# tsnorri/vcf2multialign

Hardware: AMD Instinct MI355X
Metric: aligned A2M Gbases/sec (higher is better)
Workload: dtype u8

## Files before the change

### vcf2multialign_amd/csrc/kernels.hpp

```cpp
#pragma once

#include <hip/hip_runtime.h>
#include <stdint.h>

#ifdef V2M_CHECKED_BUILD
__device__ uint32_t v2m_lds_poison_seed;
#endif

namespace v2m {

typedef uint32_t u32;
typedef uint64_t u64;

constexpr int kWave = 64;
typedef u32 vec4u __attribute__((ext_vector_type(4)));
typedef vec4u vec4u_unaligned8 __attribute__((aligned(8)));

#ifdef V2M_CHECKED_BUILD
__device__ __forceinline__ u32 poison_hash(u32 seed, u32 wg, u32 i)
{
	u32 h = seed ^ (wg * 0x9E3779B1u) ^ (i * 0x85EBCA77u);
	h ^= h >> 15; h *= 0x2C1B3C6Du;
	h ^= h >> 12; h *= 0x297A2D39u;
	h ^= h >> 15;
// ... 1065 lines not shown
		if (lane == 0) excl = 0;
		u32 const chunk_max = __shfl(incl, 63, kWave);

		u32 run = excl > cur ? excl : cur;
		bool uncertain = false;
		for (u64 m = w; m; m &= m - 1) {
			u32 const e = wi * 64u + __builtin_ctzll(m);
			edge_span const sp = spans[e];
			uncertain |= sp.src < run;
			run = sp.tgt > run ? sp.tgt : run;
		}

		u64 out = w;
		if (__any(uncertain)) {
			out = 0;
			u32 c = cur;
			u64 busy = __ballot(w != 0);
			while (busy) {
				int const j = __builtin_ctzll(busy);
				busy &= busy - 1;
				if (lane == j) {
					for (u64 m = w; m; m &= m - 1) {
						int const b = __builtin_ctzll(m);
						edge_span const sp = spans[wi * 64u + b];
						if (sp.src >= c) {
							out |= 1ULL << b;
							c = sp.tgt;
						}
					}
				}
				c = __shfl(c, j, kWave);
			}
			cur = c;
		} else {
			cur = chunk_max > cur ? chunk_max : cur;
		}
		if (wi < word_end)
			eff_row[wi] = out;
	}
}


struct tile_tables {
	u32 const *edge_begin;
	u32 const *cross_offsets;
	u32 const *cross_edges;
};

template <typename LabelPtr>
__device__ __forceinline__ void fill_patch_bytes(
	unsigned char *tile, u32 tile_base, u32 aln_begin, u32 label_len, LabelPtr label,
	u32 from, u32 to, u32 start, u32 step, char gap)
{
	for (u32 pos = from + start; pos < to; pos += step) {
		u32 const off = pos - aln_begin;
		tile[pos - tile_base] = (off < label_len) ? (unsigned char) label[off] : (unsigned char) gap;
	}
}

constexpr int kCandLds = 512;
constexpr int kLabelLds = 1024;
constexpr int kGroupRowsLds = 16;
constexpr int kEffWordsLds = kCandLds / 64 + 2;
constexpr int kLongQueueLds = 16;

struct cached_patch {
	unsigned short begin_rel;
	unsigned short span;
	unsigned short label_rel;
	unsigned short label_len;
};

struct patch_cache {
	cached_patch patch[kCandLds];
	u64 eff[kGroupRowsLds][kEffWordsLds];
	unsigned char labels[kLabelLds];
	u32 long_queue[kLongQueueLds];
	u32 long_count;
};

struct tile_job {
	u32 tile_base, tile_end;
	u32 cross_begin, n_cross, range_begin, n_range;
	u32 n_lds;
	u32 w0;
};

__device__ __forceinline__ void load_eff_cache(
	patch_cache &pc, tile_job const &job, u64 const *__restrict__ eff, u64 eff_words_per_row, u32 first_row, u32 n_rows, int t)
{
	if (0 == job.n_lds) return;
	u32 const nw = ((job.range_begin + job.n_lds - 1) >> 6) - job.w0 + 1;
	u32 const rows = n_rows < (u32) kGroupRowsLds ? n_rows : (u32) kGroupRowsLds;
	for (u32 i = t; i < rows * nw; i += kSpliceThreads)
		pc.eff[i / nw][i % nw] = eff[(u64) (first_row + i / nw) * eff_words_per_row + job.w0 + i % nw];
}

template <bool kWindow = false, bool kSet = false>
__device__ __forceinline__ void load_patch_cache(
	patch_cache &pc, tile_job &job, tile_tables const &tt, edge_patch const *__restrict__ patches, char const *__restrict__ labels,
	u64 const *__restrict__ eff, u64 eff_words_per_row, u32 tile, u32 row_begin, u32 n_group_rows, int t, u32 col_base = 0, u32 col_end = 0,
	set_tile_tables const st = set_tile_tables{})
{
	if (kSet) {
		job.tile_base = st.col_begin[tile];
		job.tile_end = st.col_end[tile];
	} else {
		job.tile_base = (kWindow ? col_base : 0u) + tile * (u32) kTileBytes;
		job.tile_end = (kWindow && col_end - job.tile_base < (u32) kTileBytes) ? col_end : job.tile_base + kTileBytes;
	}
	job.cross_begin = tt.cross_offsets[tile];
	job.n_cross = tt.cross_offsets[tile + 1] - job.cross_begin;
	job.range_begin = tt.edge_begin[tile];
	job.n_range = (kSet ? st.edge_end[tile] : tt.edge_begin[tile + 1]) - job.range_begin;
	job.n_lds = job.n_range < (u32) kCandLds ? job.n_range : (u32) kCandLds;
	job.w0 = job.range_begin >> 6;
	if (job.n_lds) {
		u32 const label_base = patches[job.range_begin].label_begin;
		for (u32 i = t; i < job.n_lds; i += kSpliceThreads) {
			edge_patch const p = patches[job.range_begin + i];
			u32 const span = p.aln_end - p.aln_begin, rel = p.label_begin - label_base;
			cached_patch c;
			c.begin_rel = (unsigned short) (p.aln_begin - job.tile_base);
			c.span = span < 0xFFFFu ? (unsigned short) span : (unsigned short) 0xFFFF;
			bool const label_ok = rel + p.label_len <= (u32) kLabelLds;
			c.label_rel = label_ok ? (unsigned short) rel : (unsigned short) 0xFFFF;
			c.label_len = label_ok ? (unsigned short) p.label_len : (unsigned short) 0;
			pc.patch[i] = c;
		}
		edge_patch const last = patches[job.range_begin + job.n_lds - 1];
		u32 const label_span = last.label_begin + last.label_len - label_base;
		u32 const label_len = label_span < (u32) kLabelLds ? label_span : (u32) kLabelLds;
		for (u32 i = t; i < label_len; i += kSpliceThreads)
			pc.labels[i] = (unsigned char) labels[label_base + i];
	}
	load_eff_cache(pc, job, eff, eff_words_per_row, row_begin, n_group_rows, t);
	if (t == 0) pc.long_count = 0;
}

struct tile_patch {
	u32 edge;
	u32 aln_begin;
	u32 from, to;
	u32 label_len;
	u32 label_begin;
	bool in_lds;
};

__device__ __forceinline__ u32 candidate_edge(tile_job const &job, tile_tables const &tt, u32 i)
{
	return (i < job.n_cross) ? tt.cross_edges[job.cross_begin + i] : job.range_begin + (i - job.n_cross);
}

__device__ __forceinline__ bool candidate_in_lds(tile_job const &job, u32 i)
{
	return i >= job.n_cross && i - job.n_cross < job.n_lds;
}

template <bool kWindow = false>
__device__ __forceinline__ tile_patch candidate_patch(
	patch_cache const &pc, tile_job const &job, edge_patch const *__restrict__ patches, u32 i, u32 e, bool cached)
{
	u32 const tile_end = kWindow ? job.tile_end : job.tile_base + kTileBytes;
	cached_patch c{};
	if (cached) {
		c = pc.patch[i - job.n_cross];
		cached = c.span != 0xFFFF && c.label_rel != 0xFFFF;
	}
	tile_patch tp;
	tp.edge = e;
	if (cached) {
		tp.aln_begin = tp.from = job.tile_base + c.begin_rel;
		tp.to = tp.from + c.span < tile_end ? tp.from + c.span : tile_end;
		tp.label_len = c.label_len;
		tp.label_begin = c.label_rel;
		tp.in_lds = true;
	} else {
		edge_patch const p = patches[e];
		tp.aln_begin = p.aln_begin;
		tp.from = p.aln_begin > job.tile_base ? p.aln_begin : job.tile_base;
		tp.to = p.aln_end < tile_end ? p.aln_end : tile_end;
		tp.label_len = p.label_len;
		tp.label_begin = p.label_begin;
		tp.in_lds = false;
	}
	return tp;
}

__device__ __forceinline__ bool candidate_effective(
	patch_cache const &pc, tile_job const &job, tile_tables const &tt, u64 const *__restrict__ eff_row, u32 local_row, u32 i,
	u32 &e, bool &cached)
{
	cached = candidate_in_lds(job, i) && local_row < (u32) kGroupRowsLds;
	if (cached) {
		e = job.range_begin + (i - job.n_cross);
		return (pc.eff[local_row][(e >> 6) - job.w0] >> (e & 63)) & 1;
	}
	e = candidate_edge(job, tt, i);
	return (eff_row[e >> 6] >> (e & 63)) & 1;
}

template <bool kWindow, typename F>
__device__ __forceinline__ void for_each_effective_candidate(
	patch_cache const &pc, tile_job const &job, tile_tables const &tt, edge_patch const *__restrict__ patches,
	u64 const *__restrict__ eff_row, u32 local_row, int t, F &&f)
{
	u32 const n_cand = job.n_cross + job.n_range;
	for (u32 i = t; i < n_cand; i += kSpliceThreads) {
		u32 e;
		bool cached;
		if (!candidate_effective(pc, job, tt, eff_row, local_row, i, e, cached)) continue;
		f(candidate_patch<kWindow>(pc, job, patches, i, e, cached));
	}
}

template <bool kWindow = false>
__device__ __forceinline__ void patch_row_tile(
	unsigned char *buf, patch_cache &pc, tile_job const &job, tile_tables const &tt,
	edge_patch const *__restrict__ patches, char const *__restrict__ labels,
	u64 const *__restrict__ eff_row, u32 local_row, int t, char gap)
{
	u32 const tile_end = kWindow ? job.tile_end : job.tile_base + kTileBytes;
	for_each_effective_candidate<kWindow>(pc, job, tt, patches, eff_row, local_row, t, [&](tile_patch const &tp) {
		if (tp.to - tp.from > kLongPatch) {
			u32 const slot = atomicAdd(&pc.long_count, 1u);
			if (slot < (u32) kLongQueueLds) { pc.long_queue[slot] = tp.edge; return; }
		}
		if (tp.in_lds)
			fill_patch_bytes(buf, job.tile_base, tp.aln_begin, tp.label_len, pc.labels + tp.label_begin, tp.from, tp.to, 0, 1, gap);
		else
			fill_patch_bytes(buf, job.tile_base, tp.aln_begin, tp.label_len, labels + tp.label_begin, tp.from, tp.to, 0, 1, gap);
	});
	__syncthreads();

	u32 const n_long = pc.long_count < (u32) kLongQueueLds ? pc.long_count : (u32) kLongQueueLds;
	if (n_long) {
		for (u32 q = t >> 6; q < n_long; q += kSpliceThreads >> 6) {
			edge_patch const p = patches[pc.long_queue[q]];
			u32 const from = p.aln_begin > job.tile_base ? p.aln_begin : job.tile_base;
			u32 const to = p.aln_end < tile_end ? p.aln_end : tile_end;
			fill_patch_bytes(buf, job.tile_base, p.aln_begin, p.label_len, labels + p.label_begin, from, to, t & 63, 64, gap);
		}
		__syncthreads();
		if (t == 0) pc.long_count = 0;
	}
	V2M_POISON_LDS_RANGE(pc.long_queue, 0u, (u32) kLongQueueLds);
}

__device__ __forceinline__ void map_block(u32 b, u32 n_groups, u32 n_tiles, u32 tile_run, u32 &tile, u32 &group)
{
	u32 const per_super = tile_run * n_groups;
	u32 const super = b / per_super, within = b % per_super;
	u32 const t0 = super * tile_run;
	u32 const run = (n_tiles - t0 < tile_run) ? n_tiles - t0 : tile_run;
	group = within / run;
	tile = t0 + within % run;
}

__device__ __forceinline__ u32 set_tile_chunks(set_tile_tables const &st, u32 tile)
{
	return (st.col_end[tile] - st.col_begin[tile] + 15u) >> 4;
}

template <bool kNonTemporal, bool kWindow, bool kSet = false>
__device__ __forceinline__ void splice_aligned_tiles(
	vec4u const *__restrict__ tmpl, u64 const *__restrict__ eff, u64 eff_words_per_row,
	tile_tables tt, edge_patch const *__restrict__ patches, char const *__restrict__ labels,
	char *__restrict__ out, u64 row_pitch, u32 n_rows, u32 rows_per_group, u32 n_groups, u32 n_tiles, u32 tile_run,
	u64 store_limit, char gap, u32 col_base, u32 col_end, set_tile_tables const st = set_tile_tables{})
{
	__shared__ vec4u lds[2][kTileChunks];
	__shared__ patch_cache pc;

	int const t = threadIdx.x;
	u32 tile, group;
	map_block(blockIdx.x, n_groups, n_tiles, tile_run, tile, group);
	u32 const row_begin = group * rows_per_group;
	u32 const row_end = (row_begin + rows_per_group < n_rows) ? row_begin + rows_per_group : n_rows;
	V2M_POISON_LDS(lds);
	V2M_POISON_LDS(pc);

	u32 const n_chunks = kSet ? set_tile_chunks(st, tile) : (u32) kTileChunks;
	u32 const record_offset = kSet ? st.record_offset[tile] : 0u;
	vec4u pristine[kChunksPerThread];
#pragma unroll
	for (int k = 0; k < kChunksPerThread; ++k) {
		if (kSet) pristine[k] = (u32) (t + kSpliceThreads * k) < n_chunks ? tmpl[(record_offset >> 4) + t + kSpliceThreads * k] : vec4u{0, 0, 0, 0};
		else pristine[k] = tmpl[(u64) tile * kTileChunks + t + kSpliceThreads * k];
	}

	tile_job job;
	load_patch_cache<kWindow, kSet>(pc, job, tt, patches, labels, eff, eff_words_per_row, tile, row_begin, row_end - row_begin, t, col_base, col_end, st);
	u32 const tile_base = job.tile_base;

	for (u32 row = row_begin; row < row_end; ++row) {
		vec4u *const buf = lds[(row - row_begin) & 1];
		u32 const cached_row = (row - row_begin) % (u32) kGroupRowsLds;
		if (row != row_begin && 0 == cached_row)
			load_eff_cache(pc, job, eff, eff_words_per_row, row, row_end - row, t);
#pragma unroll
		for (int k = 0; k < kChunksPerThread; ++k)
			if (!kSet || (u32) (t + kSpliceThreads * k) < n_chunks) buf[t + kSpliceThreads * k] = pristine[k];
		__syncthreads();

		patch_row_tile<kWindow>((unsigned char *) buf, pc, job, tt, patches, labels, eff + (u64) row * eff_words_per_row, cached_row, t, gap);

		char *const dst = out + (u64) row * row_pitch + (kSet ? (u64) record_offset : (u64) tile * kTileBytes);
#pragma unroll
		for (int k = 0; k < kChunksPerThread; ++k) {
			int const c = t + kSpliceThreads * k;
			if (kSet ? (u32) c < n_chunks : (kWindow ? (u64) tile * kTileBytes : (u64) tile_base) + (u64) c * 16 < store_limit) {
				vec4u const nv = buf[c];
				if (kNonTemporal)
					__builtin_nontemporal_store(nv, (vec4u *) (dst + c * 16));
				else
					*(vec4u *) (dst + c * 16) = nv;
			}
		}
	}
}

template <bool kNonTemporal>
__global__ __launch_bounds__(kSpliceThreads) void splice_aligned_kernel(
	vec4u const *__restrict__ tmpl, u64 const *__restrict__ eff, u64 eff_words_per_row,
	tile_tables tt, edge_patch const *__restrict__ patches, char const *__restrict__ labels,
	char *__restrict__ out, u64 row_pitch, u32 n_rows, u32 rows_per_group, u32 n_groups, u32 n_tiles, u32 tile_run,
	u64 store_limit , char gap)
{
	splice_aligned_tiles<kNonTemporal, false>(tmpl, eff, eff_words_per_row, tt, patches, labels, out, row_pitch, n_rows, rows_per_group, n_groups,
		n_tiles, tile_run, store_limit, gap, 0u, 0u);
}

template <bool kNonTemporal>
__global__ __launch_bounds__(kSpliceThreads) void splice_aligned_window_kernel(
	vec4u const *__restrict__ tmpl, u64 const *__restrict__ eff, u64 eff_words_per_row,
	tile_tables tt, edge_patch const *__restrict__ patches, char const *__restrict__ labels,
	char *__restrict__ out, u64 row_pitch, u32 n_rows, u32 rows_per_group, u32 n_groups, u32 n_tiles, u32 tile_run,
	u64 store_limit, char gap, u32 col_base, u32 col_end)
{
	splice_aligned_tiles<kNonTemporal, true>(tmpl, eff, eff_words_per_row, tt, patches, labels, out, row_pitch, n_rows, rows_per_group, n_groups,
		n_tiles, tile_run, store_limit, gap, col_base, col_end);
}

template <bool kNonTemporal>
__global__ __launch_bounds__(kSpliceThreads) void splice_aligned_set_kernel(
	vec4u const *__restrict__ tmpl, u64 const *__restrict__ eff, u64 eff_words_per_row,
	tile_tables tt, set_tile_tables st, edge_patch const *__restrict__ patches, char const *__restrict__ labels,
	char *__restrict__ out, u64 row_pitch, u32 n_rows, u32 rows_per_group, u32 n_groups, u32 n_tiles, u32 tile_run, char gap)
{
	splice_aligned_tiles<kNonTemporal, true, true>(tmpl, eff, eff_words_per_row, tt, patches, labels, out, row_pitch, n_rows, rows_per_group, n_groups,
		n_tiles, tile_run, 0, gap, 0u, 0u, st);
}


__device__ __forceinline__ u32 zero_bytes_mask(u32 x)
{
	return ~(((x & 0x7F7F7F7Fu) + 0x7F7F7F7Fu) | x | 0x7F7F7F7Fu);
}

__device__ __forceinline__ u32 wave_inclusive_scan_u32(u32 v)
{
	v += (u32) __builtin_amdgcn_update_dpp(0, (int) v, 0x111, 0xf, 0xf, false);
	v += (u32) __builtin_amdgcn_update_dpp(0, (int) v, 0x112, 0xf, 0xf, false);
	v += (u32) __builtin_amdgcn_update_dpp(0, (int) v, 0x114, 0xf, 0xf, false);
	v += (u32) __builtin_amdgcn_update_dpp(0, (int) v, 0x118, 0xf, 0xf, false);
	v += (u32) __builtin_amdgcn_update_dpp(0, (int) v, 0x142, 0xa, 0xf, false);
	v += (u32) __builtin_amdgcn_update_dpp(0, (int) v, 0x143, 0xc, 0xf, false);
	return v;
}

// ... 38 lines not shown
	u32 *__restrict__ tile_counts , u32 n_tiles,
	u32 n_rows, u32 rows_per_group, u32 n_groups, u32 tile_run, u32 col_base, u32 col_end, set_tile_tables const st = set_tile_tables{})
{
	__shared__ vec4u lds[kTileChunks];
	__shared__ patch_cache pc;
	__shared__ int row_delta[kCountRowsMax];
	__shared__ int cand_delta[kCandDeltaLds];
	__shared__ u32 wave_sums[kSpliceThreads / 64];

	int const t = threadIdx.x;
	u32 tile, group;
	map_block(blockIdx.x, n_groups, n_tiles, tile_run, tile, group);
	u32 const row_begin = group * rows_per_group;
	u32 const row_end = (row_begin + rows_per_group < n_rows) ? row_begin + rows_per_group : n_rows;
	V2M_POISON_LDS(lds);
	V2M_POISON_LDS(pc);
	V2M_POISON_LDS(row_delta);
	V2M_POISON_LDS(cand_delta);
	V2M_POISON_LDS(wave_sums);

	u32 const n_chunks = kSet ? set_tile_chunks(st, tile) : (u32) kTileChunks;
	u32 mine = 0;
#pragma unroll
	for (int k = 0; k < kChunksPerThread; ++k) {
		if (kSet && (u32) (t + kSpliceThreads * k) >= n_chunks) continue;
		vec4u const v = tmpl0[(kSet ? (u64) (st.record_offset[tile] >> 4) : (u64) tile * kTileChunks) + t + kSpliceThreads * k];
		lds[t + kSpliceThreads * k] = v;
#pragma unroll
		for (int d = 0; d < 4; ++d)
			mine += 4 - __builtin_popcount(zero_bytes_mask(v[d]));
	}
#pragma unroll
	for (int d = 32; d >= 1; d >>= 1) mine += __shfl_down(mine, d, kWave);
	if ((t & 63) == 0) wave_sums[t >> 6] = mine;
	for (u32 r = t; r < (u32) kCountRowsMax; r += kSpliceThreads) row_delta[r] = 0;

	tile_job job;
	load_patch_cache<kWindow, kSet>(pc, job, tt, patches, labels, eff, eff_words_per_row, tile, row_begin, row_end - row_begin, t, col_base, col_end, st);
	__syncthreads();
	u32 tile_count = 0;
#pragma unroll
	for (int wv = 0; wv < kSpliceThreads / 64; ++wv) tile_count += wave_sums[wv];

	unsigned char const *const tile_bytes = (unsigned char const *) lds;
	auto patch_delta = [&](tile_patch const &tp) {
		u32 const label_end = tp.aln_begin + tp.label_len;
		int const label_in_tile = label_end > tp.from ? (int) ((label_end < tp.to ? label_end : tp.to) - tp.from) : 0;
		return label_in_tile - (int) count_nonzero_bytes(tile_bytes, tp.from - job.tile_base, tp.to - job.tile_base);
	};
	u32 const n_cand = job.n_cross + job.n_range;
	for (u32 i = t; i < n_cand && i < (u32) kCandDeltaLds; i += kSpliceThreads)
		cand_delta[i] = patch_delta(candidate_patch<kWindow>(pc, job, patches, i, candidate_edge(job, tt, i), candidate_in_lds(job, i)));
	__syncthreads();
	for (u32 sub = row_begin; sub < row_end; sub += kGroupRowsLds) {
		u32 const sub_end = sub + kGroupRowsLds < row_end ? sub + kGroupRowsLds : row_end;
		if (sub != row_begin) {
			asm volatile("s_waitcnt lgkmcnt(0)" ::: "memory");
			__syncthreads();
			load_eff_cache(pc, job, eff, eff_words_per_row, sub, sub_end - sub, t);
			__syncthreads();
		}
		u32 const sub_rows = sub_end - sub;
		u32 const nw = job.n_lds ? ((job.range_begin + job.n_lds - 1) >> 6) - job.w0 + 1 : 0;
		for (u32 idx = t; idx < sub_rows * nw; idx += kSpliceThreads) {
			u32 const r = idx / nw, w = idx % nw;
			u32 const first = (job.w0 + w) * 64u;
			u64 bits = pc.eff[r][w];
			if (first < job.range_begin) bits &= ~0ULL << (job.range_begin - first);
			u32 const cached_end = job.range_begin + job.n_lds;
			if (cached_end < first + 64u) bits &= (1ULL << (cached_end - first)) - 1;
			int delta = 0;
			for (; bits; bits &= bits - 1) {
				u32 const e = first + (u32) __builtin_ctzll(bits);
				u32 const i = job.n_cross + (e - job.range_begin);
				delta += i < (u32) kCandDeltaLds ? cand_delta[i] : patch_delta(candidate_patch<kWindow>(pc, job, patches, i, e, true));
			}
			if (delta) atomicAdd(&row_delta[sub - row_begin + r], delta);
		}
		u32 const n_other = n_cand - job.n_lds;
		for (u32 idx = t; idx < sub_rows * n_other; idx += kSpliceThreads) {
			u32 const r = idx / n_other, j = idx % n_other;
			u32 const i = j < job.n_cross ? j : j + job.n_lds;
			u32 const e = candidate_edge(job, tt, i);
			if (!((eff[(u64) (sub + r) * eff_words_per_row + (e >> 6)] >> (e & 63)) & 1)) continue;
			int const delta = i < (u32) kCandDeltaLds ? cand_delta[i] : patch_delta(candidate_patch<kWindow>(pc, job, patches, i, e, false));
			if (delta) atomicAdd(&row_delta[sub - row_begin + r], delta);
		}
	}
	__syncthreads();
	for (u32 r = t; r < row_end - row_begin; r += kSpliceThreads)
		tile_counts[(u64) (row_begin + r) * n_tiles + tile] = (u32) ((int) tile_count + row_delta[r]);
}

__global__ __launch_bounds__(kSpliceThreads) void count_unaligned_kernel(
	vec4u const *__restrict__ tmpl0, u64 const *__restrict__ eff, u64 eff_words_per_row,
	tile_tables tt, edge_patch const *__restrict__ patches, char const *__restrict__ labels,
	u32 *__restrict__ tile_counts , u32 n_tiles,
	u32 n_rows, u32 rows_per_group, u32 n_groups, u32 tile_run)
{
	count_unaligned_tiles<false>(tmpl0, eff, eff_words_per_row, tt, patches, labels, tile_counts, n_tiles, n_rows, rows_per_group, n_groups, tile_run, 0u, 0u);
}

__global__ __launch_bounds__(kSpliceThreads) void count_unaligned_window_kernel(
	vec4u const *__restrict__ tmpl0, u64 const *__restrict__ eff, u64 eff_words_per_row,
	tile_tables tt, edge_patch const *__restrict__ patches, char const *__restrict__ labels,
	u32 *__restrict__ tile_counts , u32 n_tiles,
	u32 n_rows, u32 rows_per_group, u32 n_groups, u32 tile_run, u32 col_base, u32 col_end)
{
	count_unaligned_tiles<true>(tmpl0, eff, eff_words_per_row, tt, patches, labels, tile_counts, n_tiles, n_rows, rows_per_group, n_groups, tile_run, col_base, col_end);
}

__global__ __launch_bounds__(kSpliceThreads) void count_unaligned_set_kernel(
// ... 174 lines not shown
	if (c & 4) { *(u32_unaligned *) p = (u32) rest; p += 4; rest >>= 32; }
	if (c & 2) { *(u16_unaligned *) p = (u16) rest; p += 2; rest >>= 16; }
	if (c & 1) *p = (char) rest;
}

template <bool kNonTemporal, u32 kQueue, bool kWindow, bool kSet = false>
__device__ __forceinline__ void splice_unaligned_tiles(
	vec4u const *__restrict__ tmpl0, u64 const *__restrict__ eff, u64 eff_words_per_row,
	tile_tables tt, edge_patch const *__restrict__ patches, char const *__restrict__ labels,
	u32 const *__restrict__ tile_offsets , u32 n_tiles,
	char *__restrict__ out, u64 row_pitch, u32 n_rows, u32 rows_per_group, u32 n_groups, u32 tile_run, u32 col_base, u32 col_end,
	set_tile_tables const st = set_tile_tables{})
{
	constexpr int kWaves = kSpliceThreads / 64, kSlots = kChunksPerThread * kWaves;
	__shared__ vec4u lds[kTileChunks];
	__shared__ patch_cache pc;
	__shared__ __attribute__((aligned(16))) u32 wave_sums[kSlots];
	__shared__ u32 compact_sel[16];
	__shared__ vec4u queue_data[kQueue];
	__shared__ u32 queue_desc[kQueue];
	__shared__ u32 queue_count;

	V2M_POISON_LDS(lds);
	V2M_POISON_LDS(pc);
	V2M_POISON_LDS(wave_sums);
	V2M_POISON_LDS(compact_sel);
	V2M_POISON_LDS(queue_data);
	V2M_POISON_LDS(queue_desc);
	V2M_POISON_LDS(queue_count);
	int const t = threadIdx.x;
	int const lane = t & 63, wave = __builtin_amdgcn_readfirstlane(t >> 6);
	if (t < 16) compact_sel[t] = compaction_selector((u32) t);
	u32 tile, group;
	map_block(blockIdx.x, n_groups, n_tiles, tile_run, tile, group);
	{
		u32 const t0 = tile / tile_run * tile_run;
		u32 const run = (n_tiles - t0 < tile_run) ? n_tiles - t0 : tile_run;
		if (0 == run % 8) { u32 const j = tile - t0; tile = t0 + (j & 7) * (run / 8) + (j >> 3); }
	}
	u32 const row_begin = group * rows_per_group;
	u32 const row_end = (row_begin + rows_per_group < n_rows) ? row_begin + rows_per_group : n_rows;

	u32 const n_chunks = kSet ? set_tile_chunks(st, tile) : (u32) kTileChunks;
	vec4u pristine[kChunksPerThread];
#pragma unroll
	for (int k = 0; k < kChunksPerThread; ++k) {
		if (kSet) pristine[k] = (u32) (t + kSpliceThreads * k) < n_chunks ? tmpl0[(st.record_offset[tile] >> 4) + t + kSpliceThreads * k] : vec4u{0, 0, 0, 0};
		else pristine[k] = tmpl0[(u64) tile * kTileChunks + t + kSpliceThreads * k];
	}

	tile_job job;
	load_patch_cache<kWindow, kSet>(pc, job, tt, patches, labels, eff, eff_words_per_row, tile, row_begin, row_end - row_begin, t, col_base, col_end, st);

	char *dst_prev = out;
	for (u32 row = row_begin; ; ++row) {
		bool const past_end = row >= row_end;
		u32 const tile_offset = past_end ? 0u : tile_offsets[(u64) row * n_tiles + tile];
		if (!past_end) {
			if (row != row_begin && 0 == (row - row_begin) % (u32) kGroupRowsLds)
				load_eff_cache(pc, job, eff, eff_words_per_row, row, row_end - row, t);
#pragma unroll
			for (int k = 0; k < kChunksPerThread; ++k)
				if (!kSet || (u32) (t + kSpliceThreads * k) < n_chunks) lds[t + kSpliceThreads * k] = pristine[k];
		}
		asm volatile("s_waitcnt lgkmcnt(0)" ::: "memory");
		__syncthreads();

		if (row != row_begin) {
			u32 const n = (u32) __builtin_amdgcn_readfirstlane((int) queue_count);
			V2M_POISON_LDS_RANGE(queue_desc, n < kQueue ? n : kQueue, kQueue);
			V2M_POISON_LDS_RANGE(queue_data, n < kQueue ? n : kQueue, kQueue);
			for (u32 pass = 0; 64 * pass < n; ++pass) {
				if (((row + pass) & (u32) (kWaves - 1)) != (u32) wave) continue;
				u32 const idx = 64 * pass + (u32) lane;
				if (idx < n) {
					u32 const e = queue_desc[idx];
					pack_chunk_and_store_exact(queue_data[idx], e & 15u, dst_prev + (e >> 4), compact_sel);
				}
			}
		}
		if (past_end) break;

		patch_row_tile<kWindow>((unsigned char *) lds, pc, job, tt, patches, labels, eff + (u64) row * eff_words_per_row, (row - row_begin) % (u32) kGroupRowsLds, t, 0);

		vec4u v[kChunksPerThread];
		u32 mine[kChunksPerThread], incl[kChunksPerThread];
#pragma unroll
		for (int k = 0; k < kChunksPerThread; ++k) {
			if (kSet) v[k] = (u32) (t + kSpliceThreads * k) < n_chunks ? lds[t + kSpliceThreads * k] : vec4u{0, 0, 0, 0};
			else v[k] = lds[t + kSpliceThreads * k];
		}
#pragma unroll
		for (int k = 0; k < kChunksPerThread; ++k) {
			u32 bytes = 0;
#pragma unroll
			for (int d = 0; d < 4; ++d) bytes = __builtin_amdgcn_msad_u8(v[k][d] ^ 0x01010101u, v[k][d], bytes);
			incl[k] = mine[k] = bytes | (bytes - 1u < 15u ? 0x10000u : 0u);
		}
		wave_inclusive_scan_u32_lockstep(incl);
		if (lane == 63) {
			vec4u sums;
#pragma unroll
			for (int k = 0; k < kChunksPerThread; ++k) sums[k] = incl[k];
			*(vec4u *) &wave_sums[kChunksPerThread * wave] = sums;
		}
		__syncthreads();

		u32 slot_end = lane < kSlots ? wave_sums[kChunksPerThread * (lane % kWaves) + lane / kWaves] : 0u;
		slot_end += (u32) __builtin_amdgcn_update_dpp(0, (int) slot_end, 0x111, 0xf, 0xf, false);
		slot_end += (u32) __builtin_amdgcn_update_dpp(0, (int) slot_end, 0x112, 0xf, 0xf, false);
		slot_end += (u32) __builtin_amdgcn_update_dpp(0, (int) slot_end, 0x114, 0xf, 0xf, false);
		slot_end += (u32) __builtin_amdgcn_update_dpp(0, (int) slot_end, 0x118, 0xf, 0xf, false);

		char *const dst = out + (u64) row * row_pitch + tile_offset;
		u32 const n_fit = (u32) __builtin_popcountll(__ballot(lane < kSlots && (slot_end >> 16) <= kQueue));
		u32 const n_queued = n_fit ? (u32) __builtin_amdgcn_readlane((int) slot_end, (int) n_fit - 1) >> 16 : 0u;
		u32 offs[kChunksPerThread];
		u32 dense = 0;
#pragma unroll
		for (int k = 0; k < kChunksPerThread; ++k) {
			int const slot = k * kWaves + wave;
			u32 const slot_begin = slot ? (u32) __builtin_amdgcn_readlane((int) slot_end, slot - 1) : 0u;
			u32 const c = mine[k] & 0xFFFFu;
			u32 const before = slot_begin + incl[k] - mine[k];
			u32 const off = before & 0xFFFFu;
			offs[k] = off;
			if (16 == c) {
				if (kNonTemporal) __builtin_nontemporal_store(v[k], (vec4u_unaligned *) (dst + off));
				else *(vec4u_unaligned *) (dst + off) = v[k];
			}
			if ((u32) slot < n_fit) {
				if (mine[k] >> 16) {
					u32 const pos = before >> 16;
					queue_desc[pos] = c | off << 4;
					queue_data[pos] = v[k];
				}
			}
			else dense |= 1u << k;
		}
		for (; dense; dense &= dense - 1) {
			u32 const j = (u32) __builtin_ctz(dense);
			u32 const c = (0 == j ? mine[0] : 1 == j ? mine[1] : 2 == j ? mine[2] : mine[3]) & 0xFFFFu;
			u32 const o = 0 == j ? offs[0] : 1 == j ? offs[1] : 2 == j ? offs[2] : offs[3];
			if (c - 1u < 15u) pack_chunk_and_store_exact(lds[(u32) t + (u32) kSpliceThreads * j], c, dst + o, compact_sel);
		}
		if (0 == t) queue_count = n_queued;
		dst_prev = dst;
	}
}

template <bool kNonTemporal, u32 kQueue = 128>
__global__ __launch_bounds__(kSpliceThreads) void splice_unaligned_kernel(
	vec4u const *__restrict__ tmpl0, u64 const *__restrict__ eff, u64 eff_words_per_row,
	tile_tables tt, edge_patch const *__restrict__ patches, char const *__restrict__ labels,
	u32 const *__restrict__ tile_offsets , u32 n_tiles,
	char *__restrict__ out, u64 row_pitch, u32 n_rows, u32 rows_per_group, u32 n_groups, u32 tile_run)
{
	splice_unaligned_tiles<kNonTemporal, kQueue, false>(tmpl0, eff, eff_words_per_row, tt, patches, labels, tile_offsets, n_tiles, out, row_pitch,
		n_rows, rows_per_group, n_groups, tile_run, 0u, 0u);
}

template <bool kNonTemporal>
__global__ __launch_bounds__(kSpliceThreads) void splice_unaligned_window_kernel(
	vec4u const *__restrict__ tmpl0, u64 const *__restrict__ eff, u64 eff_words_per_row,
	tile_tables tt, edge_patch const *__restrict__ patches, char const *__restrict__ labels,
	u32 const *__restrict__ tile_offsets, u32 n_tiles,
	char *__restrict__ out, u64 row_pitch, u32 n_rows, u32 rows_per_group, u32 n_groups, u32 tile_run, u32 col_base, u32 col_end)
{
	splice_unaligned_tiles<kNonTemporal, 128, true>(tmpl0, eff, eff_words_per_row, tt, patches, labels, tile_offsets, n_tiles, out, row_pitch,
		n_rows, rows_per_group, n_groups, tile_run, col_base, col_end);
}

template <bool kNonTemporal>
__global__ __launch_bounds__(kSpliceThreads) void splice_unaligned_set_kernel(
	vec4u const *__restrict__ tmpl0, u64 const *__restrict__ eff, u64 eff_words_per_row,
	tile_tables tt, set_tile_tables st, edge_patch const *__restrict__ patches, char const *__restrict__ labels,
	u32 const *__restrict__ tile_offsets, u32 n_tiles,
	char *__restrict__ out, u64 row_pitch, u32 n_rows, u32 rows_per_group, u32 n_groups, u32 tile_run)
{
	splice_unaligned_tiles<kNonTemporal, 128, true, true>(tmpl0, eff, eff_words_per_row, tt, patches, labels, tile_offsets, n_tiles, out, row_pitch,
		n_rows, rows_per_group, n_groups, tile_run, 0u, 0u, st);
}

__global__ __launch_bounds__(256) void scan_tile_counts_kernel(u32 *__restrict__ tile_counts, u32 n_tiles, u64 *__restrict__ row_lengths)
{
	__shared__ u32 wave_sums[4];
	__shared__ u32 carry_s;
	u32 *const row = tile_counts + (u64) blockIdx.x * n_tiles;
	V2M_POISON_LDS(wave_sums);
	V2M_POISON_LDS(carry_s);
	int const t = threadIdx.x, lane = t & 63, wave = t >> 6;
	if (t == 0) carry_s = 0;
	__syncthreads();
	for (u32 base = 0; base < n_tiles; base += 256) {
		u32 const i = base + t;
		u32 const mine = i < n_tiles ? row[i] : 0;
		u32 const incl = wave_inclusive_scan_u32(mine);
		if (lane == 63) wave_sums[wave] = incl;
		__syncthreads();
		u32 before = carry_s, total = 0;
// ... 3 lines not shown
			if (wv < wave) before += ws;
			total += ws;
		}
		if (i < n_tiles) row[i] = before + incl - mine;
		__syncthreads();
		if (t == 0) carry_s += total;
		__syncthreads();
	}
	if (t == 0) row_lengths[blockIdx.x] = carry_s;
}


struct row_op_record { u32 cls, ref_pos, row_pos; };

__device__ __forceinline__ u32 nonzero_byte_bits(vec4u const v)
{
	u32 bits = 0;
#pragma unroll
	for (int d = 0; d < 4; ++d) {
		u32 const keep = ~zero_bytes_mask(v[d]) & 0x80808080u;
		bits |= (((keep >> 7) | (keep >> 14) | (keep >> 21) | (keep >> 28)) & 0xFu) << (4 * d);
	}
	return bits;
}

__device__ __forceinline__ u32 mismatch_byte_bits(vec4u const a, vec4u const b)
{
	u32 bits = 0;
#pragma unroll
	for (int d = 0; d < 4; ++d) {
		u32 const x = a[d] ^ b[d];
		u32 const v = a[d] | 0x20202020u, low = v & 0x7F7F7F7Fu;
		u32 const letter = (low + 0x1F1F1F1Fu) & ~(low + 0x05050505u) & ~v;
		u32 const keep = (~zero_bytes_mask(x & 0xDFDFDFDFu) | ((x << 2) & ~letter)) & 0x80808080u;
		bits |= (((keep >> 7) | (keep >> 14) | (keep >> 21) | (keep >> 28)) & 0xFu) << (4 * d);
	}
	return bits;
}

constexpr int kOpsSlots = kChunksPerThread * (kSpliceThreads / 64);

template <bool kEmit, bool kSplit>
__device__ __forceinline__ void row_ops_tiles(
	vec4u const *__restrict__ tmpl0, u64 const *__restrict__ eff, u64 eff_words_per_row,
	tile_tables tt, edge_patch const *__restrict__ patches, char const *__restrict__ labels,
	u32 *__restrict__ tile_info ,
	u32 n_tiles, u32 n_rows, u32 rows_per_group, u32 n_groups, u32 tile_run,
	u32 const *__restrict__ op_offsets , u32 const *__restrict__ tile_ref_before ,
	u32 const *__restrict__ tile_row_before , u64 const *__restrict__ op_base ,
	row_op_record *__restrict__ out, u64 out_capacity)
{
	constexpr int kWaves = kSpliceThreads / 64;
	__shared__ vec4u lds[kTileChunks];
	__shared__ patch_cache pc;
	__shared__ u32 slot_last[kOpsSlots];
	__shared__ u32 slot_sums[2][kOpsSlots];
	__shared__ u32 wave_sums[kWaves];
	__shared__ u32 first_class;

	V2M_POISON_LDS(lds);
	V2M_POISON_LDS(pc);
	V2M_POISON_LDS(slot_last);
	V2M_POISON_LDS(slot_sums);
	V2M_POISON_LDS(wave_sums);
	V2M_POISON_LDS(first_class);
	int const t = threadIdx.x;
	int const lane = t & 63, wave = __builtin_amdgcn_readfirstlane(t >> 6);
	u32 tile, group;
	map_block(blockIdx.x, n_groups, n_tiles, tile_run, tile, group);
	u32 const row_begin = group * rows_per_group;
	u32 const row_end = (row_begin + rows_per_group < n_rows) ? row_begin + rows_per_group : n_rows;

	vec4u pristine[kChunksPerThread];
	u32 ref_bits[kChunksPerThread];
#pragma unroll
	for (int k = 0; k < kChunksPerThread; ++k) {
		pristine[k] = tmpl0[(u64) tile * kTileChunks + t + kSpliceThreads * k];
		ref_bits[k] = nonzero_byte_bits(pristine[k]);
	}
	u32 const ref_before_tile = kEmit ? tile_ref_before[tile] : 0u;

	tile_job job;
	load_patch_cache<false, false>(pc, job, tt, patches, labels, eff, eff_words_per_row, tile, row_begin, row_end - row_begin, t);
	u64 const below_lanes = (1ULL << lane) - 1;

	for (u32 row = row_begin; row < row_end; ++row) {
		if (row != row_begin && 0 == (row - row_begin) % (u32) kGroupRowsLds)
			load_eff_cache(pc, job, eff, eff_words_per_row, row, row_end - row, t);
#pragma unroll
		for (int k = 0; k < kChunksPerThread; ++k) lds[t + kSpliceThreads * k] = pristine[k];
		if (!kEmit && 0 == t) first_class = 0;
		asm volatile("s_waitcnt lgkmcnt(0)" ::: "memory");
		__syncthreads();

		patch_row_tile<false>((unsigned char *) lds, pc, job, tt, patches, labels, eff + (u64) row * eff_words_per_row, (row - row_begin) % (u32) kGroupRowsLds, t, 0);

		u32 row_bits[kChunksPerThread], wave_carry[kChunksPerThread];
		u32 ne_bits[kSplit ? kChunksPerThread : 1];
#pragma unroll
		for (int k = 0; k < kChunksPerThread; ++k) {
			vec4u const mine = lds[t + kSpliceThreads * k];
			row_bits[k] = nonzero_byte_bits(mine);
			if constexpr (kSplit) ne_bits[k] = mismatch_byte_bits(pristine[k], mine) & ref_bits[k] & row_bits[k];
			u32 const live = ref_bits[k] | row_bits[k];
			u32 last = 0;
			if (live) {
				u32 const top = 31u - (u32) __builtin_clz(live);
				last = ((ref_bits[k] >> top) & 1u) | (((row_bits[k] >> top) & 1u) << 1);
				if constexpr (kSplit) last |= ((ne_bits[k] >> top) & 1u) << 2;
			}
			u64 const b0 = __ballot(last & 1u), b1 = __ballot(last & 2u);
			u64 const b2 = kSplit ? __ballot(last & 4u) : 0ULL;
			u64 const any = b0 | b1, before = any & below_lanes;
			u32 carry = 0;
			if (before) {
				u32 const p = 63u - (u32) __builtin_clzll(before);
				carry = (u32) ((b0 >> p) & 1u) | ((u32) ((b1 >> p) & 1u) << 1);
				if constexpr (kSplit) carry |= (u32) ((b2 >> p) & 1u) << 2;
			}
			wave_carry[k] = carry;
			if (0 == lane) {
				u32 slot_class = 0;
				if (any) {
					u32 const p = 63u - (u32) __builtin_clzll(any);
					slot_class = (u32) ((b0 >> p) & 1u) | ((u32) ((b1 >> p) & 1u) << 1);
					if constexpr (kSplit) slot_class |= (u32) ((b2 >> p) & 1u) << 2;
				}
				slot_last[k * kWaves + wave] = slot_class;
			}
		}
		__syncthreads();

		u32 const tile_carry = kEmit ? tile_info[(u64) row * n_tiles + tile] : 0u;
		u32 breaks[kChunksPerThread], slot_carry[kChunksPerThread];
		u32 tile_last = tile_carry;
#pragma unroll
		for (int s = 0; s < kOpsSlots; ++s) {
			if (wave == s % kWaves) slot_carry[s / kWaves] = tile_last;
			u32 const c = slot_last[s];
			if (c) tile_last = c;
		}
// ... 34 lines not shown
				u32 total = 0;
#pragma unroll
				for (int wv = 0; wv < kWaves; ++wv) total += wave_sums[wv];
				tile_info[(u64) row * n_tiles + tile] = total | first_class << 16 | tile_last << (kSplit ? 19 : 18);
			}
		} else {
			u32 mine[2 * kChunksPerThread], incl[2 * kChunksPerThread];
#pragma unroll
			for (int k = 0; k < kChunksPerThread; ++k) {
				incl[k] = mine[k] = (u32) __builtin_popcount(breaks[k]) | (u32) __builtin_popcount(ref_bits[k]) << 16;
				incl[kChunksPerThread + k] = mine[kChunksPerThread + k] = (u32) __builtin_popcount(row_bits[k]);
			}
			wave_inclusive_scan_u32_lockstep(incl);
			if (63 == lane) {
#pragma unroll
				for (int k = 0; k < kChunksPerThread; ++k) {
					slot_sums[0][k * kWaves + wave] = incl[k];
					slot_sums[1][k * kWaves + wave] = incl[kChunksPerThread + k];
				}
			}
			__syncthreads();
			u64 const row_tile = (u64) row * n_tiles + tile;
			u64 const first_op = op_base[row] + op_offsets[row_tile];
			u32 const row_before_tile = tile_row_before[row_tile];
			u32 slot_a[kChunksPerThread], slot_b[kChunksPerThread];
			{
				u32 run_a = 0, run_b = 0;
#pragma unroll
				for (int s = 0; s < kOpsSlots; ++s) {
					if (wave == s % kWaves) { slot_a[s / kWaves] = run_a; slot_b[s / kWaves] = run_b; }
					run_a += slot_sums[0][s];
					run_b += slot_sums[1][s];
				}
			}
#pragma unroll
			for (int k = 0; k < kChunksPerThread; ++k) {
				u32 const before_a = slot_a[k] + incl[k] - mine[k];
				u32 const before_b = slot_b[k] + incl[kChunksPerThread + k] - mine[kChunksPerThread + k];
				for (u32 b = breaks[k]; b; b &= b - 1) {
					u32 const i = (u32) __builtin_ctz(b), lower = (1u << i) - 1u;
					row_op_record rec;
					rec.cls = ((ref_bits[k] >> i) & 1u) | (((row_bits[k] >> i) & 1u) << 1);
					if constexpr (kSplit) rec.cls |= ((ne_bits[k] >> i) & 1u) << 2;
					rec.ref_pos = ref_before_tile + (before_a >> 16) + (u32) __builtin_popcount(ref_bits[k] & lower);
					rec.row_pos = row_before_tile + before_b + (u32) __builtin_popcount(row_bits[k] & lower);
					u64 const at = first_op + (before_a & 0xFFFFu) + (u32) __builtin_popcount(breaks[k] & lower);
					if (at < out_capacity) out[at] = rec;
				}
			}
		}
	}
}

__global__ __launch_bounds__(kSpliceThreads) void count_row_ops_kernel(
	vec4u const *__restrict__ tmpl0, u64 const *__restrict__ eff, u64 eff_words_per_row,
	tile_tables tt, edge_patch const *__restrict__ patches, char const *__restrict__ labels,
	u32 *__restrict__ tile_info , u32 n_tiles, u32 n_rows, u32 rows_per_group, u32 n_groups, u32 tile_run)
{
	row_ops_tiles<false, false>(tmpl0, eff, eff_words_per_row, tt, patches, labels, tile_info, n_tiles, n_rows, rows_per_group, n_groups, tile_run,
		nullptr, nullptr, nullptr, nullptr, nullptr, 0);
}

__global__ __launch_bounds__(kSpliceThreads) void emit_row_ops_kernel(
	vec4u const *__restrict__ tmpl0, u64 const *__restrict__ eff, u64 eff_words_per_row,
	tile_tables tt, edge_patch const *__restrict__ patches, char const *__restrict__ labels,
	u32 *__restrict__ tile_info , u32 n_tiles, u32 n_rows, u32 rows_per_group, u32 n_groups, u32 tile_run,
	u32 const *__restrict__ op_offsets, u32 const *__restrict__ tile_ref_before, u32 const *__restrict__ tile_row_before, u64 const *__restrict__ op_base,
	row_op_record *__restrict__ out, u64 out_capacity)
{
	row_ops_tiles<true, false>(tmpl0, eff, eff_words_per_row, tt, patches, labels, tile_info, n_tiles, n_rows, rows_per_group, n_groups, tile_run,
		op_offsets, tile_ref_before, tile_row_before, op_base, out, out_capacity);
}

__global__ __launch_bounds__(kSpliceThreads) void count_row_ops_eqx_kernel(
	vec4u const *__restrict__ tmpl0, u64 const *__restrict__ eff, u64 eff_words_per_row,
	tile_tables tt, edge_patch const *__restrict__ patches, char const *__restrict__ labels,
	u32 *__restrict__ tile_info , u32 n_tiles, u32 n_rows, u32 rows_per_group, u32 n_groups, u32 tile_run)
{
	row_ops_tiles<false, true>(tmpl0, eff, eff_words_per_row, tt, patches, labels, tile_info, n_tiles, n_rows, rows_per_group, n_groups, tile_run,
		nullptr, nullptr, nullptr, nullptr, nullptr, 0);
}

__global__ __launch_bounds__(kSpliceThreads) void emit_row_ops_eqx_kernel(
	vec4u const *__restrict__ tmpl0, u64 const *__restrict__ eff, u64 eff_words_per_row,
	tile_tables tt, edge_patch const *__restrict__ patches, char const *__restrict__ labels,
	u32 *__restrict__ tile_info , u32 n_tiles, u32 n_rows, u32 rows_per_group, u32 n_groups, u32 tile_run,
	u32 const *__restrict__ op_offsets, u32 const *__restrict__ tile_ref_before, u32 const *__restrict__ tile_row_before, u64 const *__restrict__ op_base,
	row_op_record *__restrict__ out, u64 out_capacity)
{
	row_ops_tiles<true, true>(tmpl0, eff, eff_words_per_row, tt, patches, labels, tile_info, n_tiles, n_rows, rows_per_group, n_groups, tile_run,
		op_offsets, tile_ref_before, tile_row_before, op_base, out, out_capacity);
}

__global__ __launch_bounds__(256) void scan_row_ops_kernel(u32 *__restrict__ tile_info, u32 *__restrict__ op_offsets, u32 n_tiles, u32 *__restrict__ n_ops)
{
	__shared__ u32 wave_sums[4];
	__shared__ u32 wave_last[4];
	__shared__ u32 carry_s[2];
	V2M_POISON_LDS(wave_sums);
	V2M_POISON_LDS(wave_last);
	V2M_POISON_LDS(carry_s);
	u32 *const info = tile_info + (u64) blockIdx.x * n_tiles;
	u32 *const offsets = op_offsets + (u64) blockIdx.x * n_tiles;
	int const t = threadIdx.x, lane = t & 63, wave = t >> 6;
	if (t == 0) { carry_s[0] = 0; carry_s[1] = 0; }
	__syncthreads();
	for (u32 base = 0; base < n_tiles; base += 256) {
// ... 515 lines not shown
```

Before: 6881.

## Cache cross-edge bits and more eff rows in LDS, restructure splice patch loops

```diff
diff --git a/vcf2multialign_amd/csrc/kernels.hpp b/vcf2multialign_amd/csrc/kernels.hpp
--- a/vcf2multialign_amd/csrc/kernels.hpp
+++ b/vcf2multialign_amd/csrc/kernels.hpp
@@ -1141,17 +1141,29 @@
 	unsigned char *tile, u32 tile_base, u32 aln_begin, u32 label_len, LabelPtr label,
 	u32 from, u32 to, u32 start, u32 step, char gap)
 {
-	for (u32 pos = from + start; pos < to; pos += step) {
-		u32 const off = pos - aln_begin;
-		tile[pos - tile_base] = (off < label_len) ? (unsigned char) label[off] : (unsigned char) gap;
-	}
+	asm volatile("" : "+s"(step));
+	u32 const label_end = aln_begin + label_len < to ? aln_begin + label_len : to;
+	u32 pos = from + start;
+#pragma clang loop unroll(disable)
+	for (; pos < label_end; pos += step)
+		tile[pos - tile_base] = (unsigned char) label[pos - aln_begin];
+#pragma clang loop unroll(disable)
+	for (; pos < to; pos += step)
+		tile[pos - tile_base] = (unsigned char) gap;
+}
+
+__device__ __forceinline__ void settle_loaded(vec4u &v)
+{
+	asm volatile("" : "+v"(v));
 }
 
 constexpr int kCandLds = 512;
 constexpr int kLabelLds = 1024;
+constexpr int kSpliceRowsLds = 32;
 constexpr int kGroupRowsLds = 16;
 constexpr int kEffWordsLds = kCandLds / 64 + 2;
 constexpr int kLongQueueLds = 16;
+constexpr int kCrossLds = 8;
 
 struct cached_patch {
 	unsigned short begin_rel;
@@ -1160,13 +1172,18 @@
 	unsigned short label_len;
 };
 
-struct patch_cache {
+template <int kRows>
+struct patch_cache_rows {
+	static constexpr int kCachedRows = kRows;
 	cached_patch patch[kCandLds];
-	u64 eff[kGroupRowsLds][kEffWordsLds];
+	u64 eff[kRows][kEffWordsLds];
 	unsigned char labels[kLabelLds];
 	u32 long_queue[kLongQueueLds];
 	u32 long_count;
+	unsigned char cross_eff[kRows];
 };
+typedef patch_cache_rows<kSpliceRowsLds> patch_cache;
+typedef patch_cache_rows<kGroupRowsLds> ops_patch_cache;
 
 struct tile_job {
 	u32 tile_base, tile_end;
@@ -1175,19 +1192,33 @@
 	u32 w0;
 };
 
+template <typename Cache>
 __device__ __forceinline__ void load_eff_cache(
-	patch_cache &pc, tile_job const &job, u64 const *__restrict__ eff, u64 eff_words_per_row, u32 first_row, u32 n_rows, int t)
-{
-	if (0 == job.n_lds) return;
-	u32 const nw = ((job.range_begin + job.n_lds - 1) >> 6) - job.w0 + 1;
-	u32 const rows = n_rows < (u32) kGroupRowsLds ? n_rows : (u32) kGroupRowsLds;
-	for (u32 i = t; i < rows * nw; i += kSpliceThreads)
-		pc.eff[i / nw][i % nw] = eff[(u64) (first_row + i / nw) * eff_words_per_row + job.w0 + i % nw];
-}
-
-template <bool kWindow = false, bool kSet = false>
+	Cache &pc, tile_job const &job, tile_tables const &tt, u64 const *__restrict__ eff, u64 eff_words_per_row, u32 first_row, u32 n_rows, int t)
+{
+	u32 const rows = n_rows < (u32) Cache::kCachedRows ? n_rows : (u32) Cache::kCachedRows;
+	if (job.n_lds) {
+		u32 const nw = ((job.range_begin + job.n_lds - 1) >> 6) - job.w0 + 1;
+		for (u32 i = t; i < rows * nw; i += kSpliceThreads)
+			pc.eff[i / nw][i % nw] = eff[(u64) (first_row + i / nw) * eff_words_per_row + job.w0 + i % nw];
+	}
+	u32 const n_cross_lds = job.n_cross < (u32) kCrossLds ? job.n_cross : (u32) kCrossLds;
+	asm volatile("" : "+v"(t));
+	u32 const r = (u32) (kSpliceThreads - 1 - t);
+	if (n_cross_lds && r < rows) {
+		u64 const *const eff_row = eff + (u64) (first_row + r) * eff_words_per_row;
+		u32 bits = 0;
+		for (u32 j = 0; j < n_cross_lds; ++j) {
+			u32 const e = tt.cross_edges[job.cross_begin + j];
+			bits |= (u32) ((eff_row[e >> 6] >> (e & 63)) & 1) << j;
+		}
+		pc.cross_eff[r] = (unsigned char) bits;
+	}
+}
+
+template <bool kWindow = false, bool kSet = false, typename Cache>
 __device__ __forceinline__ void load_patch_cache(
-	patch_cache &pc, tile_job &job, tile_tables const &tt, edge_patch const *__restrict__ patches, char const *__restrict__ labels,
+	Cache &pc, tile_job &job, tile_tables const &tt, edge_patch const *__restrict__ patches, char const *__restrict__ labels,
 	u64 const *__restrict__ eff, u64 eff_words_per_row, u32 tile, u32 row_begin, u32 n_group_rows, int t, u32 col_base = 0, u32 col_end = 0,
 	set_tile_tables const st = set_tile_tables{})
 {
@@ -1223,7 +1254,7 @@
 		for (u32 i = t; i < label_len; i += kSpliceThreads)
 			pc.labels[i] = (unsigned char) labels[label_base + i];
 	}
-	load_eff_cache(pc, job, eff, eff_words_per_row, row_begin, n_group_rows, t);
+	load_eff_cache(pc, job, tt, eff, eff_words_per_row, row_begin, n_group_rows, t);
 	if (t == 0) pc.long_count = 0;
 }
 
@@ -1236,76 +1267,97 @@
 	bool in_lds;
 };
 
-__device__ __forceinline__ u32 candidate_edge(tile_job const &job, tile_tables const &tt, u32 i)
-{
-	return (i < job.n_cross) ? tt.cross_edges[job.cross_begin + i] : job.range_begin + (i - job.n_cross);
-}
-
-__device__ __forceinline__ bool candidate_in_lds(tile_job const &job, u32 i)
-{
-	return i >= job.n_cross && i - job.n_cross < job.n_lds;
-}
-
-template <bool kWindow = false>
-__device__ __forceinline__ tile_patch candidate_patch(
-	patch_cache const &pc, tile_job const &job, edge_patch const *__restrict__ patches, u32 i, u32 e, bool cached)
+__device__ __forceinline__ bool cached_patch_usable(cached_patch const &c)
+{
+	return c.span != 0xFFFF && c.label_rel != 0xFFFF;
+}
+
+template <bool kWindow>
+__device__ __forceinline__ tile_patch lds_tile_patch(tile_job const &job, cached_patch const &c, u32 e)
 {
 	u32 const tile_end = kWindow ? job.tile_end : job.tile_base + kTileBytes;
-	cached_patch c{};
-	if (cached) {
-		c = pc.patch[i - job.n_cross];
-		cached = c.span != 0xFFFF && c.label_rel != 0xFFFF;
-	}
 	tile_patch tp;
 	tp.edge = e;
+	tp.aln_begin = tp.from = job.tile_base + c.begin_rel;
+	tp.to = tp.from + c.span < tile_end ? tp.from + c.span : tile_end;
+	tp.label_len = c.label_len;
+	tp.label_begin = c.label_rel;
+	tp.in_lds = true;
+	return tp;
+}
+
+template <bool kWindow>
+__device__ __forceinline__ tile_patch global_tile_patch(tile_job const &job, edge_patch const *__restrict__ patches, u32 e)
+{
+	u32 const tile_end = kWindow ? job.tile_end : job.tile_base + kTileBytes;
+	edge_patch const p = patches[e];
+	tile_patch tp;
+	tp.edge = e;
+	tp.aln_begin = p.aln_begin;
+	tp.from = p.aln_begin > job.tile_base ? p.aln_begin : job.tile_base;
+	tp.to = p.aln_end < tile_end ? p.aln_end : tile_end;
+	tp.label_len = p.label_len;
+	tp.label_begin = p.label_begin;
+	tp.in_lds = false;
+	return tp;
+}
+
+__device__ __forceinline__ u32 candidate_edge(tile_job const &job, tile_tables const &tt, u32 i)
+{
+	return (i < job.n_cross) ? tt.cross_edges[job.cross_begin + i] : job.range_begin + (i - job.n_cross);
+}
+
+__device__ __forceinline__ bool candidate_in_lds(tile_job const &job, u32 i)
+{
+	return i >= job.n_cross && i - job.n_cross < job.n_lds;
+}
+
+template <bool kWindow = false, typename Cache>
+__device__ __forceinline__ tile_patch candidate_patch(
+	Cache const &pc, tile_job const &job, edge_patch const *__restrict__ patches, u32 i, u32 e, bool cached)
+{
 	if (cached) {
-		tp.aln_begin = tp.from = job.tile_base + c.begin_rel;
-		tp.to = tp.from + c.span < tile_end ? tp.from + c.span : tile_end;
-		tp.label_len = c.label_len;
-		tp.label_begin = c.label_rel;
-		tp.in_lds = true;
-	} else {
-		edge_patch const p = patches[e];
-		tp.aln_begin = p.aln_begin;
-		tp.from = p.aln_begin > job.tile_base ? p.aln_begin : job.tile_base;
-		tp.to = p.aln_end < tile_end ? p.aln_end : tile_end;
-		tp.label_len = p.label_len;
-		tp.label_begin = p.label_begin;
-		tp.in_lds = false;
-	}
-	return tp;
-}
-
-__device__ __forceinline__ bool candidate_effective(
-	patch_cache const &pc, tile_job const &job, tile_tables const &tt, u64 const *__restrict__ eff_row, u32 local_row, u32 i,
-	u32 &e, bool &cached)
-{
-	cached = candidate_in_lds(job, i) && local_row < (u32) kGroupRowsLds;
-	if (cached) {
-		e = job.range_begin + (i - job.n_cross);
-		return (pc.eff[local_row][(e >> 6) - job.w0] >> (e & 63)) & 1;
-	}
-	e = candidate_edge(job, tt, i);
-	return (eff_row[e >> 6] >> (e & 63)) & 1;
-}
-
-template <bool kWindow, typename F>
+		cached_patch const c = pc.patch[i - job.n_cross];
+		if (cached_patch_usable(c)) return lds_tile_patch<kWindow>(job, c, e);
+	}
+	return global_tile_patch<kWindow>(job, patches, e);
+}
+
+template <bool kWindow, typename Cache, typename F>
 __device__ __forceinline__ void for_each_effective_candidate(
-	patch_cache const &pc, tile_job const &job, tile_tables const &tt, edge_patch const *__restrict__ patches,
+	Cache const &pc, tile_job const &job, tile_tables const &tt, edge_patch const *__restrict__ patches,
 	u64 const *__restrict__ eff_row, u32 local_row, int t, F &&f)
 {
-	u32 const n_cand = job.n_cross + job.n_range;
-	for (u32 i = t; i < n_cand; i += kSpliceThreads) {
+	bool const rows_cached = local_row < (u32) Cache::kCachedRows;
+	u32 const n_lds = rows_cached ? job.n_lds : 0u;
+	asm volatile("" : "+v"(t));
+	for (u32 j = t; j < n_lds; j += kSpliceThreads) {
+		u32 const e = job.range_begin + j;
+		if (!((pc.eff[local_row][(e >> 6) - job.w0] >> (e & 63)) & 1)) continue;
+		cached_patch const c = pc.patch[j];
+		if (cached_patch_usable(c)) f(lds_tile_patch<kWindow>(job, c, e));
+		else f(global_tile_patch<kWindow>(job, patches, e));
+	}
+
+	u32 const n_cross_lds = !rows_cached ? 0u : job.n_cross < (u32) kCrossLds ? job.n_cross : (u32) kCrossLds;
+	u32 const n_rest = job.n_cross + (job.n_range - n_lds);
+	for (u32 k = t; k < n_rest; k += kSpliceThreads) {
 		u32 e;
-		bool cached;
-		if (!candidate_effective(pc, job, tt, eff_row, local_row, i, e, cached)) continue;
-		f(candidate_patch<kWindow>(pc, job, patches, i, e, cached));
-	}
-}
-
-template <bool kWindow = false>
+		if (k < n_cross_lds) {
+			if (!((pc.cross_eff[local_row] >> k) & 1)) continue;
+			e = tt.cross_edges[job.cross_begin + k];
+			asm volatile("" : "+v"(e));
+		} else {
+			e = k < job.n_cross ? tt.cross_edges[job.cross_begin + k] : job.range_begin + n_lds + (k - job.n_cross);
+			if (!((eff_row[e >> 6] >> (e & 63)) & 1)) continue;
+		}
+		f(global_tile_patch<kWindow>(job, patches, e));
+	}
+}
+
+template <bool kWindow = false, typename Cache>
 __device__ __forceinline__ void patch_row_tile(
-	unsigned char *buf, patch_cache &pc, tile_job const &job, tile_tables const &tt,
+	unsigned char *buf, Cache &pc, tile_job const &job, tile_tables const &tt,
 	edge_patch const *__restrict__ patches, char const *__restrict__ labels,
 	u64 const *__restrict__ eff_row, u32 local_row, int t, char gap)
 {
@@ -1382,14 +1434,18 @@
 	load_patch_cache<kWindow, kSet>(pc, job, tt, patches, labels, eff, eff_words_per_row, tile, row_begin, row_end - row_begin, t, col_base, col_end, st);
 	u32 const tile_base = job.tile_base;
 
+#pragma unroll
+	for (int k = 0; k < kChunksPerThread; ++k) {
+		settle_loaded(pristine[k]);
+		if (!kSet || (u32) (t + kSpliceThreads * k) < n_chunks) lds[0][t + kSpliceThreads * k] = pristine[k];
+	}
+
 	for (u32 row = row_begin; row < row_end; ++row) {
 		vec4u *const buf = lds[(row - row_begin) & 1];
-		u32 const cached_row = (row - row_begin) % (u32) kGroupRowsLds;
+		u32 const cached_row = (row - row_begin) % (u32) kSpliceRowsLds;
 		if (row != row_begin && 0 == cached_row)
-			load_eff_cache(pc, job, eff, eff_words_per_row, row, row_end - row, t);
-#pragma unroll
-		for (int k = 0; k < kChunksPerThread; ++k)
-			if (!kSet || (u32) (t + kSpliceThreads * k) < n_chunks) buf[t + kSpliceThreads * k] = pristine[k];
+			load_eff_cache(pc, job, tt, eff, eff_words_per_row, row, row_end - row, t);
+		asm volatile("s_waitcnt lgkmcnt(0)" ::: "memory");
 		__syncthreads();
 
 		patch_row_tile<kWindow>((unsigned char *) buf, pc, job, tt, patches, labels, eff + (u64) row * eff_words_per_row, cached_row, t, gap);
@@ -1405,6 +1461,13 @@
 				else
 					*(vec4u *) (dst + c * 16) = nv;
 			}
+		}
+
+		if (row + 1 < row_end) {
+			vec4u *const next = lds[(row + 1 - row_begin) & 1];
+#pragma unroll
+			for (int k = 0; k < kChunksPerThread; ++k)
+				if (!kSet || (u32) (t + kSpliceThreads * k) < n_chunks) next[t + kSpliceThreads * k] = pristine[k];
 		}
 	}
 }
@@ -1549,12 +1612,12 @@
 	for (u32 i = t; i < n_cand && i < (u32) kCandDeltaLds; i += kSpliceThreads)
 		cand_delta[i] = patch_delta(candidate_patch<kWindow>(pc, job, patches, i, candidate_edge(job, tt, i), candidate_in_lds(job, i)));
 	__syncthreads();
-	for (u32 sub = row_begin; sub < row_end; sub += kGroupRowsLds) {
-		u32 const sub_end = sub + kGroupRowsLds < row_end ? sub + kGroupRowsLds : row_end;
+	for (u32 sub = row_begin; sub < row_end; sub += kSpliceRowsLds) {
+		u32 const sub_end = sub + kSpliceRowsLds < row_end ? sub + kSpliceRowsLds : row_end;
 		if (sub != row_begin) {
 			asm volatile("s_waitcnt lgkmcnt(0)" ::: "memory");
 			__syncthreads();
-			load_eff_cache(pc, job, eff, eff_words_per_row, sub, sub_end - sub, t);
+			load_eff_cache(pc, job, tt, eff, eff_words_per_row, sub, sub_end - sub, t);
 			__syncthreads();
 		}
 		u32 const sub_rows = sub_end - sub;
@@ -1835,17 +1898,18 @@
 	tile_job job;
 	load_patch_cache<kWindow, kSet>(pc, job, tt, patches, labels, eff, eff_words_per_row, tile, row_begin, row_end - row_begin, t, col_base, col_end, st);
 
+#pragma unroll
+	for (int k = 0; k < kChunksPerThread; ++k) {
+		settle_loaded(pristine[k]);
+		if (!kSet || (u32) (t + kSpliceThreads * k) < n_chunks) lds[t + kSpliceThreads * k] = pristine[k];
+	}
+
 	char *dst_prev = out;
 	for (u32 row = row_begin; ; ++row) {
 		bool const past_end = row >= row_end;
 		u32 const tile_offset = past_end ? 0u : tile_offsets[(u64) row * n_tiles + tile];
-		if (!past_end) {
-			if (row != row_begin && 0 == (row - row_begin) % (u32) kGroupRowsLds)
-				load_eff_cache(pc, job, eff, eff_words_per_row, row, row_end - row, t);
-#pragma unroll
-			for (int k = 0; k < kChunksPerThread; ++k)
-				if (!kSet || (u32) (t + kSpliceThreads * k) < n_chunks) lds[t + kSpliceThreads * k] = pristine[k];
-		}
+		if (!past_end && row != row_begin && 0 == (row - row_begin) % (u32) kSpliceRowsLds)
+			load_eff_cache(pc, job, tt, eff, eff_words_per_row, row, row_end - row, t);
 		asm volatile("s_waitcnt lgkmcnt(0)" ::: "memory");
 		__syncthreads();
 
@@ -1864,7 +1928,7 @@
 		}
 		if (past_end) break;
 
-		patch_row_tile<kWindow>((unsigned char *) lds, pc, job, tt, patches, labels, eff + (u64) row * eff_words_per_row, (row - row_begin) % (u32) kGroupRowsLds, t, 0);
+		patch_row_tile<kWindow>((unsigned char *) lds, pc, job, tt, patches, labels, eff + (u64) row * eff_words_per_row, (row - row_begin) % (u32) kSpliceRowsLds, t, 0);
 
 		vec4u v[kChunksPerThread];
 		u32 mine[kChunksPerThread], incl[kChunksPerThread];
@@ -1929,6 +1993,11 @@
 		}
 		if (0 == t) queue_count = n_queued;
 		dst_prev = dst;
+		if (row + 1 < row_end) {
+#pragma unroll
+			for (int k = 0; k < kChunksPerThread; ++k)
+				if (!kSet || (u32) (t + kSpliceThreads * k) < n_chunks) lds[t + kSpliceThreads * k] = pristine[k];
+		}
 	}
 }
 
@@ -2038,7 +2107,7 @@
 {
 	constexpr int kWaves = kSpliceThreads / 64;
 	__shared__ vec4u lds[kTileChunks];
-	__shared__ patch_cache pc;
+	__shared__ ops_patch_cache pc;
 	__shared__ u32 slot_last[kOpsSlots];
 	__shared__ u32 slot_sums[2][kOpsSlots];
 	__shared__ u32 wave_sums[kWaves];
@@ -2072,7 +2141,7 @@
 
 	for (u32 row = row_begin; row < row_end; ++row) {
 		if (row != row_begin && 0 == (row - row_begin) % (u32) kGroupRowsLds)
-			load_eff_cache(pc, job, eff, eff_words_per_row, row, row_end - row, t);
+			load_eff_cache(pc, job, tt, eff, eff_words_per_row, row, row_end - row, t);
 #pragma unroll
 		for (int k = 0; k < kChunksPerThread; ++k) lds[t + kSpliceThreads * k] = pristine[k];
 		if (!kEmit && 0 == t) first_class = 0;
@@ -2213,7 +2282,11 @@
 	}
 }
 
+#ifdef V2M_CHECKED_BUILD
 __global__ __launch_bounds__(kSpliceThreads) void count_row_ops_kernel(
+#else
+__global__ __launch_bounds__(kSpliceThreads, 7) void count_row_ops_kernel(
+#endif
 	vec4u const *__restrict__ tmpl0, u64 const *__restrict__ eff, u64 eff_words_per_row,
 	tile_tables tt, edge_patch const *__restrict__ patches, char const *__restrict__ labels,
 	u32 *__restrict__ tile_info , u32 n_tiles, u32 n_rows, u32 rows_per_group, u32 n_groups, u32 tile_run)
```

After: 6878. About the same (-0.0%).
